# CobaltCrabby/ray_tracer

Measured on AMD Instinct MI355X. Metric: Mrays/s (reference-semantics closest-hit queries) at 1920x1080 Sponza, higher is better.
Workload: dtype f32; 1 GPU; sponza (synthetic-262267-tris), 1920x1080, 8 spp/step, bounceLimit 8, rows interleaved over 1 GPU(s), up to 10 steps in flight per rank (groups of 10+9+9+9); scene=sponza, assets=synthetic-262267-tris, width=1920, height=1080, frames_in_flight=10, pipeline=multi-kernel (k_trace_pw + k_shade per round)

## Files before the change

ray_tracer_amd/csrc/rt_device.hip:

```cpp

#include "rt_kernels.hip.h"
#include "bvh_build.hip.h"

#include <dlfcn.h>
#include <rccl/rccl.h>

#include <algorithm>
#include <chrono>
#include <cmath>
#include <cstdio>
#include <cstdlib>
#include <string>
#include <type_traits>
#include <vector>

namespace {

struct DevBuf {
    void* p = nullptr;
    size_t bytes = 0;
    DevBuf() = default;
    DevBuf(DevBuf&& o) noexcept : p(o.p), bytes(o.bytes) { o.p = nullptr; o.bytes = 0; }
    ~DevBuf() { release(); }
    void release() { if (p) (void)hipFree(p); p = nullptr; bytes = 0; }
};

struct EventPair { hipEvent_t a, b; };
#define RT_MAX_LANES 4
#define RT_FRAMES_MAX_SLOTS (24ull << 20)
struct RowsOf {
    uint32_t width = 0, height = 0, row0 = 0, rowStride = 0, nRows = 0;
    bool whole(uint32_t w, uint32_t h) const { return width == w && height == h && row0 == 0 && rowStride == 1 && nRows == h; }
};

}

struct rt_ctx {
    std::string error;
    int device = 0, numCUs = 256;
    hipStream_t ownStream = nullptr, stream = nullptr;
    DevScene sc{};
    std::vector<DevBuf> sceneBufs;
    DevBuf texelBuf, texInfoBuf, triUVBuf, objTreeBuf, objCostBuf;
    DevBuf matBuf, sphereBuf, sphereMatBuf, objInvBuf, objFwdBuf, objMetaBuf, objBoxBuf, objSkipBuf, maskBoxBuf, emitBuf, emitPreBuf;
    SceneSources host;
    DevBuf objAlphaBuf;
    uint32_t maxLeafDepth = 0;
    std::vector<RootInfo> rootOf;
    bool cull = false;
    ncclComm_t comm = nullptr;
    int commRanks = 0, commRank = 0;
    DevBuf gatherBuf;
    DevBuf stateBuf, queueBuf, fbBuf, counterBuf, scratchBuf;
    DevBuf overflowBuf[RT_MAX_LANES];
    hipStream_t sideStream[RT_MAX_LANES - 1] = {};
    hipEvent_t forkEvent = nullptr, joinEvent[RT_MAX_LANES - 1] = {}, pollEventSide[RT_MAX_LANES - 1] = {};
    uint32_t capacity = 0;
    PathState ps{}; Queues q{};
    uint32_t* hostCounts = nullptr;
    uint32_t fbPixels = 0; bool fbValid = false;
    bool profiling = false;
    std::vector<EventPair> evPool;
    size_t evUsed = 0;
    hipEvent_t profBase = nullptr;
    DevCounters* snap = nullptr;
    hipEvent_t snapEvent = nullptr;
    hipEvent_t pollEvent = nullptr;
    DevBuf probeBuf;
    DevBuf waveTimeBuf;
    DevBuf aovBuf, aovCounterBuf;
    DevBuf shadeStatBuf;
    uint32_t aovPixels = 0; bool aovValid = false;
    RowsOf fbRows, aovRows;
    DevBuf dnWorkBuf, dnHostBuf, dnOutBuf;
// ... 347 lines not shown
    c->meas.snapSeg = seg;
    c->meas.snapPaths = paths;
}
void request_ray_cost(rt_ctx* c) {
    if (c->meas.snapPending) return;
    if (hipMemcpyAsync(c->snap, c->counterBuf.p, sizeof(DevCounters), hipMemcpyDeviceToHost, c->stream) != hipSuccess) return;
    if (hipEventRecord(c->snapEvent, c->stream) != hipSuccess) return;
    c->meas.snapPending = true;
}
void measured_new_scene(rt_ctx* c) {
    if (c->meas.snapPending) { c->meas.snapBox = c->snap->boxTests; c->meas.snapRays = c->snap->raysTraced; c->meas.snapPending = false; }
    c->meas.boxPerRay = -1.0;
}

int harvest_events(rt_ctx* c) {
    for (size_t i = 0; i < c->evUsed; i++) {
        float ms = 0.f;
        RT_HIP(c, hipEventElapsedTime(&ms, c->evPool[i].a, c->evPool[i].b));
        c->rep.traceMs += ms;
        c->rep.traceLaunches++;
        float t0 = 0.f;
        if (c->profBase && hipEventElapsedTime(&t0, c->profBase, c->evPool[i].a) == hipSuccess) c->rep.traceSpans.emplace_back(t0, t0 + ms);
    }
    c->evUsed = 0;
    return 0;
}

int rebuild_emitters(rt_ctx* c) {
    c->sc.emitCount = 0; c->sc.emitSphereMask = 0; c->sc.emitMode = 0;
    const MapLayout maps = layout_maps(c->host, c->sc.texCount);
    int rc = upload_table(c, c->objAlphaBuf, maps.objAlpha, c->sc.objAlpha);
    if (rc) return rc;
    c->sc.mapFlags = maps.mapFlags;
    if (!c->tune.lightQueries) return 0;
    const EmitterLayout e = layout_emitters(c->host, c->rootOf, c->sc.texCount);
    if (!e.mode) return 0;
    if (!e.tris.empty()) {
        if ((rc = upload_table(c, c->emitBuf, e.tris, c->sc.emitTris))) return rc;
    } else {
        if ((rc = dev_alloc(c, c->emitBuf, 256))) return rc;
        c->sc.emitTris = (const uint2*)c->emitBuf.p;
    }
    if ((rc = dev_alloc(c, c->emitPreBuf, std::max<size_t>(e.tris.size(), 1) * 4 * sizeof(float4)))) return rc;
    if (!e.tris.empty()) {
        hipLaunchKernelGGL(k_emit_precompute, dim3(((uint32_t)e.tris.size() + 63u) / 64u), dim3(64), 0, c->stream, c->sc.triPos, c->sc.emitTris, (uint32_t)e.tris.size(), (float4*)c->emitPreBuf.p);
        RT_HIP(c, hipGetLastError());
        RT_HIP(c, hipStreamSynchronize(c->stream));
    }
    c->sc.emitPre = (const float4*)c->emitPreBuf.p;
    c->sc.emitCount = (uint32_t)e.tris.size();
    c->sc.emitSphereMask = e.sphereMask;
    c->sc.emitMode = 1;
    return 0;
}

int set_materials(rt_ctx* c, const RayMaterial* m, uint32_t n) {
    int rc = upload_table(c, c->matBuf, layout_materials(m, n), c->sc.mats);
    if (rc) return rc;
    c->sc.materialCount = n;
    c->host.mats.assign(m, m + n);
    return rebuild_emitters(c);
}

int set_spheres(rt_ctx* c, const Sphere* s, uint32_t n) {
    const SphereLayout l = layout_spheres(s, n);
    int rc = upload_table(c, c->sphereBuf, l.spheres, c->sc.spheres);
    if (rc) return rc;
    if ((rc = upload_table(c, c->sphereMatBuf, l.mat, c->sc.sphereMat))) return rc;
    c->sc.sphereCount = n;
    c->sc.sphereTestMask = l.testMask;
    c->host.sphereMat.assign(l.mat.begin(), l.mat.begin() + n);
    return rebuild_emitters(c);
}

int set_objects(rt_ctx* c, const ObjectLayout& l, const RenderObject* o, uint32_t n) {
    if (l.treeLevels && getenv("RT_DEBUG_OBJTREE")) dump_object_tree(l, n);
    int rc;
    if ((rc = upload_table(c, c->objInvBuf, l.inv, c->sc.objInv))) return rc;
    if ((rc = upload_table(c, c->objFwdBuf, l.fwd, c->sc.objFwd))) return rc;
    if ((rc = upload_table(c, c->objMetaBuf, l.meta, c->sc.objMeta))) return rc;
    if ((rc = upload_table(c, c->objBoxBuf, l.box, c->sc.objBox))) return rc;
    if ((rc = upload_table(c, c->maskBoxBuf, l.maskBox, c->sc.maskBox))) return rc;
    if ((rc = upload_table(c, c->objSkipBuf, l.skipCost, c->sc.objSkipCost))) return rc;
    if ((rc = upload_table(c, c->objTreeBuf, l.tree, c->sc.objTree))) return rc;
    if ((rc = upload_table(c, c->objCostBuf, l.cost, c->sc.objCost))) return rc;
    for (int k = 0; k <= RT_OBJTREE_LEVELS; k++) c->sc.objTreeOff[k] = l.treeOff[k];
    c->sc.objTreeLevels = l.treeLevels;
    c->sc.reachCount = l.reachCount;
    c->sc.maskBase = l.maskBase;
    c->sc.cullOriginLimit = l.cullOriginLimit;
    c->cull = l.cull;
    c->sc.objectCount = n;
    c->host.objMat.resize(n); c->host.objRoot.resize(n); c->host.objSampler.resize(n);
    for (uint32_t i = 0; i < n; i++) { c->host.objMat[i] = o[i].materialIndex; c->host.objRoot[i] = o[i].bvhIndex; c->host.objSampler[i] = o[i].samplerIndex; }
    return rebuild_emitters(c);
}

}

extern "C" {

int rt_device_count(int* out) {
    int n = 0;
    hipError_t e = hipGetDeviceCount(&n);
    if (out) *out = (e == hipSuccess) ? n : 0;
    return e == hipSuccess ? 0 : -1;
}

int rt_create(int device, rt_ctx** out) {
    if (!out) return -1;
    *out = nullptr;
    int n = 0;
    if (hipGetDeviceCount(&n) != hipSuccess || n <= 0) return -2;
    if (device < 0 || device >= n) return -3;
    if (hipSetDevice(device) != hipSuccess) return -4;
    rt_ctx* c = new rt_ctx();
    c->device = device;
    if (hipStreamCreateWithFlags(&c->ownStream, hipStreamNonBlocking) != hipSuccess) { c->ownStream = nullptr; rt_destroy(c); return -5; }
    c->stream = c->ownStream;
    {
        hipDeviceProp_t prop;
        if (hipGetDeviceProperties(&prop, device) == hipSuccess && prop.multiProcessorCount > 0) c->numCUs = prop.multiProcessorCount;
    }
    if (hipHostMalloc((void**)&c->hostCounts, 64, hipHostMallocDefault) != hipSuccess) { c->hostCounts = nullptr; rt_destroy(c); return -6; }
    if (hipHostMalloc((void**)&c->snap, sizeof(DevCounters), hipHostMallocDefault) != hipSuccess) { c->snap = nullptr; rt_destroy(c); return -6; }
    if (hipEventCreateWithFlags(&c->snapEvent, hipEventDisableTiming) != hipSuccess) { c->snapEvent = nullptr; rt_destroy(c); return -6; }
    if (hipEventCreateWithFlags(&c->pollEvent, hipEventDisableTiming) != hipSuccess) { c->pollEvent = nullptr; rt_destroy(c); return -6; }
// ... 185 lines not shown
    for (int l = 0; l < nLanes; l++) {
        const uint32_t u = units / (uint32_t)nLanes + ((uint32_t)l < units % (uint32_t)nLanes ? 1u : 0u);
        const uint32_t end = std::min(nSlots, at + u * unit);
        lane[l] = Lane{d, l ? c->pollEventSide[l - 1] : c->pollEvent, at, end - at, end - at, 0, false, end == at};
        lane[l].d.stream = l ? c->sideStream[l - 1] : c->stream; lane[l].d.counts = c->q.counts + 16 * l; lane[l].d.part = l;
        at = end;
    }
    const int gridPct = part_grid_pct(c->tune, nLanes, lane[0].n);
    for (int l = 0; l < nLanes; l++) lane[l].d.gridPct = gridPct;
}

int render_rounds(rt_ctx* c, const FrameParams& fp, Lane* lane, int nLanes) {
    DevCounters* dc = (DevCounters*)c->counterBuf.p;
    int rc = 0;
    if (nLanes > 1) {
        RT_HIP(c, hipEventRecord(c->forkEvent, c->stream));
        for (int l = 1; l < nLanes; l++) RT_HIP(c, hipStreamWaitEvent(lane[l].d.stream, c->forkEvent, 0));
    }
    const uint64_t maxRounds = (uint64_t)fp.samples * ((uint64_t)fp.bounceLimit + 1);
    for (uint64_t it = 0; it < maxRounds; it++) {
        bool any = false;
        for (int l = 0; l < nLanes; l++) {
            Lane& L = lane[l];
            if (L.done) continue;
            any = true;
            const hipStream_t stream = L.d.stream; uint32_t* const counts = L.d.counts;
            const int cur = L.cur, nxt = cur ^ 1;
            uint32_t* const active[2] = {c->q.active[0] + L.begin, c->q.active[1] + L.begin};
            uint32_t* const rays[2] = {c->q.rays[0] + 3 * (size_t)L.begin, c->q.rays[1] + 3 * (size_t)L.begin};
            hipLaunchKernelGGL(k_zero_counts, dim3(1), dim3(64), 0, stream, counts + nxt, counts + 2 + nxt, counts + 4, counts + 5 + nxt, counts + 7 + nxt);
            TraceArgs ta{rays[cur], counts + 2 + cur, nullptr, nullptr, dc, counts + 5 + cur, counts + 7 + cur, L.n};
            const uint64_t ubRays = std::min<uint64_t>((uint64_t)L.ubActive * 3, (uint64_t)L.n * 3);
            if ((rc = launch_trace(c, L.d, (uint32_t)ubRays, ta))) break;
            ShadeArgs sa{active[cur], counts + cur, active[nxt], rays[nxt], counts + nxt, counts + 2 + nxt, (ShadeStatStripe*)c->shadeStatBuf.p, counts + 5 + nxt, counts + 7 + nxt, L.n};
            if (L.d.sc.mapFlags & (RT_MAP_METALNESS | RT_MAP_BUMP)) hipLaunchKernelGGL(k_shade_maps, dim3((L.ubActive + RT_BLOCK - 1) / RT_BLOCK), dim3(RT_BLOCK), 0, stream, L.d.sc, c->ps, sa, fp);
            else hipLaunchKernelGGL(k_shade, dim3((L.ubActive + RT_BLOCK - 1) / RT_BLOCK), dim3(RT_BLOCK), 0, stream, L.d.sc, c->ps, sa, fp);
            L.cur = nxt;
            if (L.pollPending && hipEventQuery(L.poll) == hipSuccess) {
                L.pollPending = false;
                L.ubActive = std::min(L.ubActive, c->hostCounts[8 + l]);
                if (L.ubActive == 0) { L.done = true; continue; }
            }
            if (!L.pollPending && (it & 7u) == 7u) {
                if (hipMemcpyAsync(c->hostCounts + 8 + l, counts + L.cur, 4, hipMemcpyDeviceToHost, stream) == hipSuccess &&
                    hipEventRecord(L.poll, stream) == hipSuccess)
                    L.pollPending = true;
            }
        }
        if (!any || rc) break;
    }
    for (int l = 1; l < nLanes; l++) {
        RT_HIP(c, hipEventRecord(c->joinEvent[l - 1], lane[l].d.stream));
        RT_HIP(c, hipStreamWaitEvent(c->stream, c->joinEvent[l - 1], 0));
    }
    hipLaunchKernelGGL(k_fold_shade_stats, dim3(1), dim3(RT_STAT_STRIPES), 0, c->stream, (ShadeStatStripe*)c->shadeStatBuf.p, dc);
    return rc;
}

int render_parts(rt_ctx* c, const FrameParams& fp, const Dispatch& d, uint32_t nSlots, float4* fb) {
    const int nLanes = ensure_part_streams(c, choose_parts(c->tune, d, c->cull, c->meas.boxPerRay, fp.samples, nSlots));
    c->rep.lastParts = nLanes;
    Lane lane[RT_MAX_LANES];
    slice_parts(c, d, nSlots, fp.nFrames, nLanes, lane);
    for (int l = 0; l < nLanes; l++) {
        const Lane& L = lane[l];
        if (!L.n) continue;
        hipLaunchKernelGGL(k_raygen, dim3((L.n + RT_BLOCK - 1) / RT_BLOCK), dim3(RT_BLOCK), 0, c->stream, d.sc, c->ps,
// ... 862 lines not shown
```

ray_tracer_amd/csrc/rt_kernels.hip.h:

```cpp
#pragma once

#include <hip/hip_runtime.h>
#include <stdint.h>

#include "rt_amd.h"
#include "rt_det_math.h"
#include "rt_probe.h"
#include "scene_layout.h"

#define RT_WAVE 64
#ifndef RT_QUEUE_ORDER
#define RT_QUEUE_ORDER 0
#endif
#ifndef RT_TE_REG
#define RT_TE_REG 1
#endif
#ifndef RT_OBJTREE
#define RT_OBJTREE 1
#endif
#ifndef RT_SHADE_IDENT
#define RT_SHADE_IDENT 1
#endif
#ifndef RT_FUSED_MAPS_BLOCKS
#define RT_FUSED_MAPS_BLOCKS 4
#endif
#define RT_BLOCK 256
#define RT_HIT_NONE 0xffffffffu
#define RT_HIT_SPHERE 0x80000000u

struct DevScene {
    const float4* nodes;
    const float4* nodesPk;
    const uint32_t* leafFirst;
    const float4* triPos;
    const float4* triNrm;
// ... 57 lines not shown
struct Queues {
    uint32_t* active[2];
    uint32_t* rays[2];
    uint32_t* counts;
};

struct FrameParams {
    float camRot[16];
    float camPos[3];
    float planeWidth, planeHeight;
    float bottomLeft[3];
    uint32_t width, height, row0, rowStride, nRows, nPixels;
    uint32_t tiled;
    uint32_t startingSeed;
    uint32_t samples, bounceLimit;
    uint32_t progressive, frameCount;
    uint32_t camReuse;
    uint32_t nFrames;
    int32_t debug;
    uint32_t boxCap, triCap;
    EnvironmentData env;
};

struct DevCounters {
    unsigned long long boxTests, triTests, raysTraced, raysHit, raysReference, paths, segments, emitterTests;
    unsigned long long skippedBoxTests;
};

#define RT_STAT_STRIPES 256u
struct ShadeStatStripe {
    unsigned long long raysReference, paths, segments, emitterTests;
    unsigned long long pad[12];
};

#define RT_AS_CONSTANT __attribute__((address_space(4)))
#define RT_AS_GLOBAL __attribute__((address_space(1)))
#define RT_AS_LDS __attribute__((address_space(3)))
typedef float rt_f4v __attribute__((ext_vector_type(4)));
typedef float rt_f2v __attribute__((ext_vector_type(2)));
template <typename T> __device__ __forceinline__ const T* rt_uniform(const T* p) { return (const T*)(const RT_AS_CONSTANT T*)(unsigned long long)p; }
template <typename T> __device__ __forceinline__ const T* rt_global(const T* p) { return (const T*)(const RT_AS_GLOBAL T*)(unsigned long long)p; }

__device__ __forceinline__ rt_vec3 f4xyz(float4 v) { return rt_v3(v.x, v.y, v.z); }
__device__ __forceinline__ float4 mk4(rt_vec3 v, float w) { return make_float4(v.x, v.y, v.z, w); }
__device__ __forceinline__ float4 mk4u(rt_vec3 v, uint32_t w) { return make_float4(v.x, v.y, v.z, __uint_as_float(w)); }

__device__ __forceinline__ rt_vec3 xform_dir_rows(float4 r0, float4 r1, float4 r2, rt_vec3 v) {
    return rt_v3((r0.x * v.x + r0.y * v.y) + r0.z * v.z, (r1.x * v.x + r1.y * v.y) + r1.z * v.z,
                 (r2.x * v.x + r2.y * v.y) + r2.z * v.z);
}
__device__ __forceinline__ rt_vec3 xform_point_rows(float4 r0, float4 r1, float4 r2, rt_vec3 v) {
    return rt_v3(((r0.x * v.x + r0.y * v.y) + r0.z * v.z) + r0.w, ((r1.x * v.x + r1.y * v.y) + r1.z * v.z) + r1.w,
                 ((r2.x * v.x + r2.y * v.y) + r2.z * v.z) + r2.w);
}

__device__ __forceinline__ uint32_t lane_id() { return __lane_id(); }
__device__ __forceinline__ uint32_t lanes_below(unsigned long long m) {
    return __builtin_amdgcn_mbcnt_hi((uint32_t)(m >> 32), __builtin_amdgcn_mbcnt_lo((uint32_t)m, 0u));
}
__device__ __forceinline__ unsigned long long wave_sum_u64(unsigned long long v) {
#pragma unroll
    for (int o = 32; o > 0; o >>= 1) v += __shfl_xor(v, o, RT_WAVE);
    return v;
}
__device__ __forceinline__ uint32_t wave_sum_u32(uint32_t v) {
#pragma unroll
// ... 748 lines not shown
    trace_pw_block<STACK, OVF, PIX, STATS, CULL, HOT, BLOCKS == 5, false>(sc, ps, ta);
}
template <bool PIX>
__global__ __launch_bounds__(RT_BLOCK, 4) void k_trace_pw_alpha(DevScene sc, PathState ps, TracePwArgs ta) {
    trace_pw_block<24, true, PIX, false, true, 0, true, true>(sc, ps, ta);
}

struct FullHit {
    rt_vec3 hitPoint, normal;
    uint32_t materialIndex;
    bool frontFace;
    float u, v;
};

__device__ __forceinline__ rt_vec3 albedo_texel(const DevScene& sc, uint32_t slot, uint32_t tri, uint32_t obj, rt_vec3 ro, rt_vec3 rd) {
    float bu, bv, bw;
    {
        const float4 i0 = rt_global(sc.objInv)[3 * obj], i1 = rt_global(sc.objInv)[3 * obj + 1], i2 = rt_global(sc.objInv)[3 * obj + 2];
        const float4 p0 = rt_global(sc.triPos)[3 * (size_t)tri], p1 = rt_global(sc.triPos)[3 * (size_t)tri + 1], p2 = rt_global(sc.triPos)[3 * (size_t)tri + 2];
        const TriHit h = tri_intersect(xform_point_rows(i0, i1, i2, ro), xform_dir_rows(i0, i1, i2, rd), f4xyz(p0), f4xyz(p1), f4xyz(p2), __float_as_uint(p0.w) != 0u);
        bu = h.u; bv = h.v; bw = h.w;
    }
    const float4 a = rt_global(sc.triUV)[2 * (size_t)tri], b = rt_global(sc.triUV)[2 * (size_t)tri + 1];
    float u = (bw * a.x + bu * a.z) + bv * b.x, v = (bw * a.y + bu * a.w) + bv * b.y;
    const bool e01 = a.x == a.z && a.y == a.w, e12 = a.z == b.x && a.w == b.y, e20 = b.x == a.x && b.y == a.y;
    if (e01 || e12 || e20) { u = 0.5f; v = 0.5f; }
    const uint4 ti = rt_global(sc.texInfo)[slot];
    const bool clampEdge = ((rt_global(sc.objMeta)[obj].w >> RT_OBJ_SAMPLER_SHIFT) & RT_OBJ_SAMPLER_MASK) == 1u;
    const uint32_t x = rt_tex_index(u, ti.y, clampEdge), y = rt_tex_index(1.f - v, ti.z, clampEdge);
    const uint32_t t = rt_global(sc.texels)[(size_t)ti.x + (size_t)y * ti.y + x];
    return rt_v3(rt_srgb8_to_linear(t & 0xffu), rt_srgb8_to_linear((t >> 8) & 0xffu), rt_srgb8_to_linear((t >> 16) & 0xffu));
}

template <bool MAPS = false>
__device__ __forceinline__ FullHit reconstruct_hit(const DevScene& sc, rt_vec3 ro, rt_vec3 rd, uint32_t obj, uint32_t tri) {
    FullHit f;
    f.u = 0.f; f.v = 0.f;
    if (obj & RT_HIT_SPHERE) {
        uint32_t i = obj & ~RT_HIT_SPHERE;
        float4 s = rt_global(sc.spheres)[i];
        SphereHit h = sphere_intersect(s, ro, rd);
        f.hitPoint = rt_add(ro, rt_scale(rd, h.dst));
        f.normal = rt_scale(rt_normalize(rt_sub(f.hitPoint, f4xyz(s))), h.frontFace ? 1.f : -1.f);
        f.materialIndex = rt_global(sc.sphereMat)[i];
        f.frontFace = h.frontFace;
        return f;
    }
    const uint4 meta = rt_global(sc.objMeta)[obj];
    const bool ident = RT_SHADE_IDENT && (meta.w & RT_OBJ_FWD_IDENTITY) && ray_is_plain(ro, rd);
    rt_vec3 trd = rd, tro = ro;
    if (!ident) {
        const float4* inv = rt_global(sc.objInv) + 3 * obj;
        const float4 i0 = inv[0], i1 = inv[1], i2 = inv[2];
        trd = xform_dir_rows(i0, i1, i2, rd);
        tro = xform_point_rows(i0, i1, i2, ro);
    }
    const float4* tp = rt_global(sc.triPos) + 3 * (size_t)tri;
    float4 a = tp[0], b = tp[1], c = tp[2];
    TriHit h = tri_intersect(tro, trd, f4xyz(a), f4xyz(b), f4xyz(c), __float_as_uint(a.w) != 0u);
    const float4* tn = rt_global(sc.triNrm) + 3 * (size_t)tri;
    rt_vec3 n0 = f4xyz(tn[0]), n1 = f4xyz(tn[1]), n2 = f4xyz(tn[2]);
    rt_vec3 ni = rt_add(rt_add(rt_scale(n0, h.w), rt_scale(n1, h.u)), rt_scale(n2, h.v));
    if (MAPS) {
        const HitUV q = hit_uv(sc, tri, h.u, h.v, h.w);
        f.u = q.u; f.v = q.v;
        const uint32_t bumpSlot = __float_as_uint(rt_global(sc.mats)[3 * meta.z + 2].w);
// ... 24 lines not shown
__device__ __forceinline__ uint32_t hit_material(const DevScene& sc, uint32_t obj) {
    return (obj & RT_HIT_SPHERE) ? rt_global(sc.sphereMat)[obj & ~RT_HIT_SPHERE] : rt_global(sc.objMeta)[obj].z;
}

__device__ __forceinline__ float schlick(float cosine, float ri) {
    float r0 = (1.f - ri) / (1.f + ri);
    r0 = r0 * r0;
    return r0 + (1.f - r0) * rt_pow(1.f - cosine, 5.f);
}

__device__ __forceinline__ rt_vec3 environment_light(const EnvironmentData& env, rt_vec3 d) {
    if (!(env.lightDir[3] == 1.f)) return rt_v3(0.f, 0.f, 0.f);
    float skyT = rt_pow(rt_smoothstep(0.f, 0.4f, -d.y), 0.35f);
    rt_vec3 sky = rt_v3(rt_mix(env.horizonColor[0], env.zenithColor[0], skyT), rt_mix(env.horizonColor[1], env.zenithColor[1], skyT),
                        rt_mix(env.horizonColor[2], env.zenithColor[2], skyT));
    rt_vec3 negL = rt_v3(-env.lightDir[0], -env.lightDir[1], -env.lightDir[2]);
    float sun = rt_pow(rt_max(0.f, rt_dot(d, negL)), env.horizonColor[3]) * env.zenithColor[3];
    float g2s = rt_smoothstep(-0.01f, 0.f, -d.y);
    float sunMask = g2s >= 1.f ? 1.f : 0.f;
    float add = sun * sunMask;
    return rt_v3(rt_mix(env.groundColor[0], sky.x, g2s) + add, rt_mix(env.groundColor[1], sky.y, g2s) + add,
                 rt_mix(env.groundColor[2], sky.z, g2s) + add);
}

__device__ __forceinline__ float light_cos(rt_vec3 dir) { return rt_dot(rt_v3(0.f, -1.f, 0.f), dir); }
__device__ __forceinline__ float light_sample_pdf(const DevScene& sc, float t, uint32_t obj, float cosTheta) {
    if (obj == RT_HIT_NONE) return 0.f;
    uint32_t m = hit_material(sc, obj);
    if (rt_global(sc.mats)[3 * m + 1].w == 0.f) return 0.f;
    float sq = t * t;
    return sq / (cosTheta * 0.4444444f);
}

__device__ __forceinline__ rt_vec3 primary_dir(const FrameParams& fp, uint32_t gx, uint32_t gy) {
    float u = (float)gx / (float)fp.width;
    float v = (float)gy / (float)fp.height;
    rt_vec3 point = rt_add(rt_v3(fp.bottomLeft[0], fp.bottomLeft[1], fp.bottomLeft[2]),
                           rt_v3(fp.planeWidth * u, fp.planeHeight * v, 0.f));
    rt_vec3 dir = rt_normalize(point);
    return rt_xform_point(fp.camRot, dir);
}

__device__ __forceinline__ uint32_t slot_frame(const FrameParams& fp, uint32_t slot) { return (slot >> 6) % fp.nFrames; }
__device__ __forceinline__ uint32_t slot_in_tile(const FrameParams& fp, uint32_t slot) { return ((slot >> 6) / fp.nFrames << 6) | (slot & 63u); }
__device__ __forceinline__ uint32_t frame_slot(const FrameParams& fp, uint32_t frame, uint32_t tileSlot) {
    return ((tileSlot >> 6) * fp.nFrames + frame) * 64u + (tileSlot & 63u);
}

__device__ __forceinline__ void slot_to_pixel(const FrameParams& fp, uint32_t slot, uint32_t& gx, uint32_t& gy, uint32_t& k) {
    if (fp.nFrames > 1u) slot = slot_in_tile(fp, slot);
    const uint32_t tiledSlots = fp.tiled ? (fp.nRows & ~7u) * fp.width : 0u;
    if (slot < tiledSlots) {
        const uint32_t tile = slot >> 6, in = slot & 63u;
        const uint32_t tilesPerRow = fp.width >> 3;
        const uint32_t tyb = tile / tilesPerRow, txb = tile - tyb * tilesPerRow;
        gx = (txb << 3) + (in & 7u);
        k = (tyb << 3) + (in >> 3);
    } else {
        k = slot / fp.width;
        gx = slot - k * fp.width;
    }
    gy = fp.row0 + k * fp.rowStride;
}

__device__ __forceinline__ void init_path(const DevScene& sc, const PathState& ps, const FrameParams& fp, uint32_t slot) {
    uint32_t gx, gy;
// ... 13 lines not shown
    ps.total()[slot] = make_float4(0.f, 0.f, 0.f, __uint_as_float(0u));
    ps.accum()[slot] = make_float4(0.f, 0.f, 0.f, 0.f);
    ps.statBox()[slot] = 0;
    ps.statTri()[slot] = 0;
}

#define RT_QUEUE_HOLE 0xffffffffu
__global__ __launch_bounds__(RT_BLOCK) void k_raygen(DevScene sc, PathState ps, uint32_t* activeOut, uint32_t* raysOut, FrameParams fp,
                                                     uint32_t slotBegin, uint32_t slotEnd) {
    const uint32_t pos = blockIdx.x * RT_BLOCK + threadIdx.x;
    const uint32_t slot = slotBegin + pos;
    if (slot >= slotEnd) return;
    if (fp.nFrames > 1u && slot_in_tile(fp, slot) >= fp.nPixels) {
        activeOut[pos] = RT_QUEUE_HOLE;
        raysOut[pos] = RT_QUEUE_HOLE;
        return;
    }
    init_path(sc, ps, fp, slot);
    activeOut[pos] = slot;
    raysOut[pos] = slot << 2;
}

struct ShadeArgs {
    const uint32_t* inActive;
    const uint32_t* inCount;
    uint32_t* outActive;
    uint32_t* outRays;
    uint32_t* outActiveCount;
    uint32_t* outRayCount;
    ShadeStatStripe* stats;
    uint32_t* outAuxCount;
    uint32_t* outAuxCount2;
    uint32_t auxOffset;
};

template <bool MAPS = false, bool QUEUED = false>
__device__ __forceinline__ void shade_path(const DevScene& sc, const PathState& ps, const FrameParams& fp, uint32_t slot, bool& alive,
                                           uint32_t& auxMask, uint32_t& refRays, uint32_t& nPaths, uint32_t& emitTests, bool withMask = true) {
    bool wantAux = false;
    auxMask = 0;
    rt_vec3 auxOrigin = rt_v3(0, 0, 0), auxL = auxOrigin, auxC = auxOrigin;
    rt_vec3 auxAlbedo = auxOrigin;
    float auxNdotL = 0.f, auxCosPdfL = 0.f, auxCosPdfC = 0.f;
    float auxCosL = 0.f, auxCosC = 0.f;
    const float4 sO = ps.rayO()[slot], sD = ps.rayD()[slot], sA = ps.att()[slot], sT = ps.total()[slot];
    const float4 hM = (QUEUED && fp.camReuse && (__float_as_uint(sA.w) & 0x0fffffffu) == 0u && __float_as_uint(sT.w) != 0u) ? ps.camHit()[slot]
                                                                                                                        : ps.hit(RAY_MAIN)[slot];
    rt_vec3 ro = f4xyz(sO), rd = f4xyz(sD);
    rt_vec3 att = f4xyz(sA), total = f4xyz(sT);
    float misW = sO.w;
    uint32_t state = __float_as_uint(sD.w);
    uint32_t jraw = __float_as_uint(sA.w);
    uint32_t samplesDone = __float_as_uint(sT.w);
    uint32_t j = jraw & 0x0fffffffu;
    const bool pending = (jraw >> 31) != 0u;
    rt_vec3 direct = (jraw & 0x40000000u) ? rt_v3(-1.f, -1.f, -1.f) : rt_v3(0.f, 0.f, 0.f);
    bool specular = false;

    const uint32_t obj = __float_as_uint(hM.y);
    const uint32_t hitTriIdx = __float_as_uint(hM.z);
    refRays = 1;
    if (fp.camReuse && j == 0u && samplesDone == 0u) ps.camHit()[slot] = hM;

    bool done = false;
    bool zeroed = false;

    if (obj != RT_HIT_NONE) {
        if (pending) {
            float4 hL = make_float4(RT_MISS_DST, __uint_as_float(RT_HIT_NONE), 0.f, 0.f), hC = hL;
            if (!(jraw & 0x20000000u)) hL = ps.hit(RAY_NEE)[slot];
            if (!(jraw & 0x10000000u)) hC = ps.hit(RAY_PROBE)[slot];
            const float4 pM = ps.pendMis()[slot];
            float tL = hL.x, tC = hC.x;
            uint32_t oL = __float_as_uint(hL.y), oC = __float_as_uint(hC.y);
            uint32_t lm = (oL == RT_HIT_NONE) ? 0u : hit_material(sc, oL);
            float4 lmE = rt_global(sc.mats)[3 * lm + 1];
            float realLightPDF = light_sample_pdf(sc, tL, oL, pM.x);
            float cosinePDF = pM.z;
            float misWeight1 = realLightPDF * realLightPDF / (realLightPDF * realLightPDF + cosinePDF * cosinePDF);
            if (rt_isnan(misWeight1)) misWeight1 = 0.f;
            float lightPDF = light_sample_pdf(sc, tC, oC, pM.y);
            float realCosinePDF = pM.w;
            float misWeight2 = realCosinePDF * realCosinePDF / (lightPDF * lightPDF + realCosinePDF * realCosinePDF);
            if (rt_isnan(misWeight2)) misWeight2 = 0.f;
            const float4 pA = ps.pendAlbedo()[slot];
            rt_vec3 albedo = f4xyz(pA);
            rt_vec3 dl = rt_scale(rt_v3(lmE.x, lmE.y, lmE.z), lmE.w);
            float k = (realLightPDF == 0.f) ? 0.f : misWeight1 / realLightPDF;
            rt_vec3 f = rt_scale(rt_scale(rt_scale(albedo, RT_INV_PI), pA.w), k);
            direct = rt_mul(dl, f);
            misW = misWeight2;
        }

        FullHit hit = reconstruct_hit<MAPS>(sc, ro, rd, obj, hitTriIdx);
        const float4* mp = rt_global(sc.mats) + 3 * hit.materialIndex;
        float4 mA = mp[0], mE = mp[1], mI = mp[2];
        if (MAPS) {
            const uint32_t metalSlot = __float_as_uint(mI.z);
            if (metalSlot < sc.texCount && !(obj & RT_HIT_SPHERE))
                mA.w = rt_srgb8_to_linear(map_red8(sc, metalSlot, ((rt_global(sc.objMeta)[obj].w >> RT_OBJ_SAMPLER_SHIFT) & RT_OBJ_SAMPLER_MASK) == 1u, hit.u, hit.v, false, false));
        }

        rt_vec3 emission = rt_scale(rt_v3(mE.x, mE.y, mE.z), mE.w);
        emission = rt_v3(emission.x / misW, emission.y / misW, emission.z / misW);
        rt_vec3 finalLight = direct.x == -1.f ? emission : direct;
        total = rt_add(total, rt_mul(finalLight, att));
        if (j == 0) total = rt_add(total, emission);
        if (rt_isnan(total.x) || rt_isnan(total.y) || rt_isnan(total.z) || total.x < 0.f || total.y < 0.f || total.z < 0.f) {
            done = true;
            zeroed = true;
        } else {
            rt_vec3 sampledDir, radiance;
            float originSign = 1.f;
            bool diffuse = false;
            if (mA.w != 0.f) {
                sampledDir = rt_reflect(rd, hit.normal);
                radiance = rt_v3(1.f, 1.f, 1.f);
                specular = true;
// ... 122 lines not shown
                if (auxMask & 2u) ps.auxDC()[slot] = mk4(auxC, 0.f);
                ps.pendAlbedo()[slot] = mk4(auxAlbedo, auxNdotL);
                ps.pendMis()[slot] = make_float4(auxCosL, auxCosC, auxCosPdfL, auxCosPdfC);
            }
        }
        const uint32_t answered = wantAux ? (((auxMask & 1u) ? 0u : 0x20000000u) | ((auxMask & 2u) ? 0u : 0x10000000u)) : 0u;
        ps.rayO()[slot] = mk4(ro, misW);
        ps.rayD()[slot] = mk4u(rd, state);
        ps.att()[slot] = mk4u(att, j | (wantAux ? 0x80000000u : 0u) | (specular ? 0x40000000u : 0u) | answered);
        const float4 nT = mk4u(total, samplesDone);
        if (!QUEUED || __float_as_uint(nT.x) != __float_as_uint(sT.x) || __float_as_uint(nT.y) != __float_as_uint(sT.y) ||
            __float_as_uint(nT.z) != __float_as_uint(sT.z) || __float_as_uint(nT.w) != __float_as_uint(sT.w))
            ps.total()[slot] = nT;
    }
}

template <bool MAPS>
__device__ __forceinline__ void shade_block(const DevScene& sc, const PathState& ps, const ShadeArgs& sa, const FrameParams& fp) {
    __shared__ uint32_t s_cnt[RT_BLOCK / RT_WAVE][8];
    __shared__ uint32_t s_base[4];
    const uint32_t n = *sa.inCount;
    if (blockIdx.x * RT_BLOCK >= n) return;
    const uint32_t gid = blockIdx.x * RT_BLOCK + threadIdx.x;
    const bool live = gid < n;

    bool alive = false;
    uint32_t auxMask = 0;
    uint32_t slot = 0;
    uint32_t refRays = 0, nPaths = 0, emitTests = 0;
    bool path = live;
    if (live) {
        slot = sa.inActive[gid];
        path = slot != 0xffffffffu;
        if (path) shade_path<MAPS, true>(sc, ps, fp, slot, alive, auxMask, refRays, nPaths, emitTests);
    }

    const unsigned long long mAlive = __ballot(alive), mM = __ballot(alive && !(auxMask & 4u));
    const unsigned long long mL = __ballot(alive && (auxMask & 1u)), mC = __ballot(alive && (auxMask & 2u));
    const uint32_t nAlive = __popcll(mAlive), nM = __popcll(mM), nL = __popcll(mL), nC = __popcll(mC);
    const uint32_t wRef = wave_sum_u32(refRays), wPaths = wave_sum_u32(nPaths), wSeg = wave_sum_u32(path ? 1u : 0u), wEmit = wave_sum_u32(emitTests);
    const uint32_t wv = threadIdx.x / RT_WAVE;
    if (lane_id() == 0) {
        s_cnt[wv][0] = nAlive; s_cnt[wv][1] = nM; s_cnt[wv][2] = wRef; s_cnt[wv][3] = wPaths; s_cnt[wv][4] = wSeg; s_cnt[wv][5] = wEmit; s_cnt[wv][6] = nL; s_cnt[wv][7] = nC;
    }
    __syncthreads();
    if (threadIdx.x == 0) {
        uint32_t tA = 0, tR = 0, tRef = 0, tP = 0, tS = 0, tE = 0, tX = 0, tY = 0;
        for (int w = 0; w < RT_BLOCK / RT_WAVE; w++) { tA += s_cnt[w][0]; tR += s_cnt[w][1]; tRef += s_cnt[w][2]; tP += s_cnt[w][3]; tS += s_cnt[w][4]; tE += s_cnt[w][5]; tX += s_cnt[w][6]; tY += s_cnt[w][7]; }
        s_base[0] = tA ? atomicAdd(sa.outActiveCount, tA) : 0u;
        s_base[1] = tR ? atomicAdd(sa.outRayCount, tR) : 0u;
        s_base[2] = tX ? atomicAdd(RT_QUEUE_ORDER ? sa.outAuxCount2 : sa.outAuxCount, tX) : 0u;
        s_base[3] = tY ? atomicAdd(RT_QUEUE_ORDER ? sa.outAuxCount : sa.outAuxCount2, tY) : 0u;
        ShadeStatStripe* const st = sa.stats + (blockIdx.x & (RT_STAT_STRIPES - 1u));
        atomicAdd(&st->raysReference, (unsigned long long)tRef);
        if (tP) atomicAdd(&st->paths, (unsigned long long)tP);
        atomicAdd(&st->segments, (unsigned long long)tS);
        if (tE) atomicAdd(&st->emitterTests, (unsigned long long)tE);
    }
    __syncthreads();
    if (alive) {
        uint32_t baseA = s_base[0], baseR = s_base[1];
        uint32_t baseX = (RT_QUEUE_ORDER ? 2u : 1u) * sa.auxOffset + s_base[2], baseY = (RT_QUEUE_ORDER ? 1u : 2u) * sa.auxOffset + s_base[3];
        for (uint32_t w = 0; w < wv; w++) { baseA += s_cnt[w][0]; baseR += s_cnt[w][1]; baseX += s_cnt[w][6]; baseY += s_cnt[w][7]; }
        sa.outActive[baseA + lanes_below(mAlive)] = slot;
        if (!(auxMask & 4u)) sa.outRays[baseR + lanes_below(mM)] = (slot << 2) | ((auxMask & 8u) ? RAY_MAIN_BLANK : (uint32_t)RAY_MAIN);
        if (auxMask & 1u) sa.outRays[baseX + lanes_below(mL)] = (slot << 2) | RAY_NEE;
        if (auxMask & 2u) sa.outRays[baseY + lanes_below(mC)] = (slot << 2) | RAY_PROBE;
    }
}

__global__ __launch_bounds__(RT_BLOCK) void k_shade(DevScene sc, PathState ps, ShadeArgs sa, FrameParams fp) { shade_block<false>(sc, ps, sa, fp); }
__global__ __launch_bounds__(RT_BLOCK) void k_shade_maps(DevScene sc, PathState ps, ShadeArgs sa, FrameParams fp) { shade_block<true>(sc, ps, sa, fp); }

__device__ __forceinline__ rt_vec3 blend_frame(const FrameParams& fp, uint32_t frameCount, float4 oldc, float4 accum) {
    rt_vec3 out = f4xyz(accum);
    float fs = (float)fp.samples;
    out = rt_v3(out.x / fs, out.y / fs, out.z / fs);
    float weight = 1.f / ((float)frameCount + 1.f);
    rt_vec3 blended = rt_add(rt_scale(rt_v3(oldc.x, oldc.y, oldc.z), 1.f - weight), rt_scale(out, weight));
    rt_vec3 fin = fp.progressive ? blended : out;
    if (rt_isnan(fin.x) || rt_isnan(fin.y) || rt_isnan(fin.z) || rt_isinf(fin.x) || rt_isinf(fin.y) || rt_isinf(fin.z))
        fin = rt_v3(1.f, 0.f, 1.f);
    return fin;
}

__device__ __forceinline__ void resolve_pixel(const PathState& ps, const FrameParams& fp, float4* rgba, uint32_t slot) {
    uint32_t gx, gy, krow;
    slot_to_pixel(fp, slot, gx, gy, krow);
    const size_t px = (size_t)krow * fp.width + gx;
    rt_vec3 fin = blend_frame(fp, fp.frameCount, rgba[px], ps.accum()[slot]);
// ... 334 lines not shown
```

ray_tracer_amd/csrc/scene_layout.cpp:

```cpp

#include "scene_layout.h"

#include <algorithm>
#include <cmath>
#include <cstdio>
#include <cstring>
#include <utility>

#include "rt_det_math.h"

namespace {

float4 with_w(float x, float y, float z, uint32_t w) {
    float4 v = make_float4(x, y, z, 0.f);
    memcpy(&v.w, &w, 4);
    return v;
}

void rows_of(const float* m, float4* out) {
    for (int r = 0; r < 3; r++) out[r] = make_float4(m[0 + r], m[4 + r], m[8 + r], m[12 + r]);
}

bool rows_are_identity(const float4* rows) {
    static const float ident[12] = {1, 0, 0, 0, 0, 1, 0, 0, 0, 0, 1, 0};
// ... 294 lines not shown
}

TextureLayout layout_textures(const RtTexture* tex, uint32_t n) {
    TextureLayout l;
    if (n > (uint32_t)RT_MAX_TEXTURES) { l.error = "more than RT_MAX_TEXTURES textures"; return l; }
    l.info.assign(std::max(n, 1u), make_uint4(0u, 1u, 1u, 0u));
    size_t total = 0;
    for (uint32_t i = 0; i < n; i++) {
        if (!tex[i].rgba8 || tex[i].width == 0 || tex[i].height == 0) { l.error = "texture " + std::to_string(i) + " is empty"; return l; }
        if ((uint64_t)tex[i].width * tex[i].height > (1ull << 28) || total + (size_t)tex[i].width * tex[i].height > 0xffffffffull) { l.error = "textures too large"; return l; }
        l.info[i] = make_uint4((uint32_t)total, tex[i].width, tex[i].height, 0u);
        total += (size_t)tex[i].width * tex[i].height;
    }
    l.texels.assign(std::max<size_t>(total, 1), 0u);
    for (uint32_t i = 0; i < n; i++) memcpy(&l.texels[l.info[i].x], tex[i].rgba8, (size_t)tex[i].width * tex[i].height * 4);
    return l;
}

MapLayout layout_maps(const SceneSources& src, uint32_t texCount) {
    MapLayout l;
    const uint32_t n = (uint32_t)src.objMat.size();
    auto bound = [&](int32_t index) { return index >= 0 && (uint32_t)index < texCount; };
    l.objAlpha.assign(std::max(n, 1u), RT_OBJALPHA_NONE);
    for (uint32_t i = 0; i < n; i++) {
        if (src.objMat[i] >= src.mats.size()) continue;
        const RayMaterial& m = src.mats[src.objMat[i]];
        if (bound(m.metalnessIndex)) l.mapFlags |= RT_MAP_METALNESS;
        if (bound(m.bumpIndex)) l.mapFlags |= RT_MAP_BUMP;
        if (bound(m.alphaIndex)) { l.mapFlags |= RT_MAP_ALPHA; l.objAlpha[i] = (uint32_t)m.alphaIndex | (src.objSampler[i] == 1u ? RT_OBJALPHA_CLAMP : 0u); }
    }
    return l;
}

EmitterLayout layout_emitters(const SceneSources& src, const std::vector<RootInfo>& rootOf, uint32_t texCount) {
    const EmitterLayout none;
    EmitterLayout l;
    if (src.mats.empty()) return none;
    auto emissive = [&](uint32_t m) { return m < src.mats.size() && !(src.mats[m].emissionStrength == 0.f); };
    for (const RayMaterial& m : src.mats)
        for (int k = 0; k < 3; k++)
            if (!std::isfinite(m.emissionColor[k] * m.emissionStrength)) return none;
    for (size_t i = 0; i < src.sphereMat.size() && i < 32; i++)
        if (emissive(src.sphereMat[i])) l.sphereMask |= 1u << i;
    for (size_t i = 32; i < src.sphereMat.size(); i++)
        if (emissive(src.sphereMat[i])) return none;
    for (size_t i = 0; i < src.objMat.size(); i++) {
        if (!emissive(src.objMat[i])) continue;
        { const int32_t ai = src.mats[src.objMat[i]].alphaIndex; if (ai >= 0 && (uint32_t)ai < texCount) return none; }
        const RootInfo& r = rootOf[src.objRoot[i]];
        if (r.triTotal == 0xffffffffu || l.tris.size() + r.triTotal > (size_t)RT_EMIT_MAX_TRIS) return none;
        for (uint32_t t = 0; t < r.triTotal; t++) l.tris.push_back(make_uint2((uint32_t)i, r.triFirst + t));
    }
    l.mode = 1;
    return l;
}
```

ray_tracer_amd/csrc/scene_layout.h:

```cpp
#pragma once

#include <hip/hip_vector_types.h>
#include <stdint.h>

#include <string>
#include <vector>

#include "rt_amd.h"

#define RT_LEAF_BIT 0x80000000u
#define RT_LEAF_CNT_SHIFT 28
#define RT_LEAF_IDX_MASK 0x0fffffffu
#define RT_HOT_PAIRS 192u
#define RT_OBJTREE_LEVELS 8

#define RT_OBJ_IDENTITY 1u
#define RT_OBJ_BOX 2u
#define RT_OBJ_MASKABLE 4u
#define RT_OBJ_FWD_IDENTITY 8u
#define RT_OBJ_SAMPLER_SHIFT 16
#define RT_OBJ_SAMPLER_MASK 0xffffu
#define RT_OBJALPHA_NONE 0xffffffffu
#define RT_OBJALPHA_SLOT_MASK 0xffu
#define RT_OBJALPHA_CLAMP 0x100u
// ... 24 lines not shown
    bool cull = false;
};
ObjectLayout layout_objects(const RenderObject* o, uint32_t n, const std::vector<RootInfo>& rootOf, uint32_t materialCount,
                            int objTreeMin, int maskIdentity);
void dump_object_tree(const ObjectLayout& l, uint32_t n);

struct SceneLayout {
    std::string error;
    MeshLayout meshes;
    ObjectLayout objects;
};
SceneLayout layout_scene(const RtSceneArrays& s, int objTreeMin, int maskIdentity);

std::vector<float4> layout_materials(const RayMaterial* m, uint32_t n);

struct SphereLayout {
    std::vector<float4> spheres;
    std::vector<uint32_t> mat;
    uint32_t testMask = 0;
};
SphereLayout layout_spheres(const Sphere* s, uint32_t n);

struct TextureLayout {
    std::string error;
    std::vector<uint4> info;
    std::vector<uint32_t> texels;
};
TextureLayout layout_textures(const RtTexture* tex, uint32_t n);

struct SceneSources {
    std::vector<RayMaterial> mats;
    std::vector<uint32_t> sphereMat, objMat, objRoot, objSampler;
};
struct MapLayout {
    std::vector<uint32_t> objAlpha;
    uint32_t mapFlags = 0;
};
MapLayout layout_maps(const SceneSources& src, uint32_t texCount);

struct EmitterLayout {
    uint32_t mode = 0, sphereMask = 0;
    std::vector<uint2> tris;
};
EmitterLayout layout_emitters(const SceneSources& src, const std::vector<RootInfo>& rootOf, uint32_t texCount);
```

Before: 4718 Mrays/s.

## Index emission by hit id and prefetch pending NEE data in queued shade

Adds a host-built per-hit emission table, appended to the material buffer, indexed directly by object or sphere hit id. This lets the queued shade path skip the hit-to-material indirection before reading emission. It also issues the pending NEE, probe, MIS and albedo loads early through branchless address selection, and spreads the per-block counter and statistics atomics across eight threads instead of one. The cost is an extra table upload on every scene change and possible extra loads of a dummy array for non-pending slots.

```diff
diff --git a/ray_tracer_amd/csrc/rt_device.hip b/ray_tracer_amd/csrc/rt_device.hip
--- a/ray_tracer_amd/csrc/rt_device.hip
+++ b/ray_tracer_amd/csrc/rt_device.hip
@@ -40,6 +40,7 @@
     int device = 0, numCUs = 256;
     hipStream_t ownStream = nullptr, stream = nullptr;
     DevScene sc{};
+    HitEmission hitEmit{};
     std::vector<DevBuf> sceneBufs;
     DevBuf texelBuf, texInfoBuf, triUVBuf, objTreeBuf, objCostBuf;
     DevBuf matBuf, sphereBuf, sphereMatBuf, objInvBuf, objFwdBuf, objMetaBuf, objBoxBuf, objSkipBuf, maskBoxBuf, emitBuf, emitPreBuf;
@@ -453,6 +454,12 @@
     int rc = upload_table(c, c->objAlphaBuf, maps.objAlpha, c->sc.objAlpha);
     if (rc) return rc;
     c->sc.mapFlags = maps.mapFlags;
+    const HitEmissionLayout hm = layout_hit_emission(c->host);
+    std::vector<float4> mats = layout_materials(c->host.mats.data(), (uint32_t)c->host.mats.size());
+    const size_t hitBase = mats.size();
+    mats.insert(mats.end(), hm.emit.begin(), hm.emit.end());
+    if ((rc = upload_table(c, c->matBuf, mats, c->sc.mats))) return rc;
+    c->hitEmit = HitEmission{c->sc.mats + hitBase, hm.sphereBase, hm.none};
     if (!c->tune.lightQueries) return 0;
     const EmitterLayout e = layout_emitters(c->host, c->rootOf, c->sc.texCount);
     if (!e.mode) return 0;
@@ -476,11 +483,13 @@
 }
 
 int set_materials(rt_ctx* c, const RayMaterial* m, uint32_t n) {
-    int rc = upload_table(c, c->matBuf, layout_materials(m, n), c->sc.mats);
-    if (rc) return rc;
+    std::vector<RayMaterial> before = c->host.mats;
+    const uint32_t countBefore = c->sc.materialCount;
     c->sc.materialCount = n;
-    c->host.mats.assign(m, m + n);
-    return rebuild_emitters(c);
+    sources_set_materials(c->host, m, n);
+    const int rc = rebuild_emitters(c);
+    if (rc) { c->host.mats.swap(before); c->sc.materialCount = countBefore; }
+    return rc;
 }
 
 int set_spheres(rt_ctx* c, const Sphere* s, uint32_t n) {
@@ -490,7 +499,7 @@
     if ((rc = upload_table(c, c->sphereMatBuf, l.mat, c->sc.sphereMat))) return rc;
     c->sc.sphereCount = n;
     c->sc.sphereTestMask = l.testMask;
-    c->host.sphereMat.assign(l.mat.begin(), l.mat.begin() + n);
+    sources_set_spheres(c->host, s, n);
     return rebuild_emitters(c);
 }
 
@@ -512,8 +521,7 @@
     c->sc.cullOriginLimit = l.cullOriginLimit;
     c->cull = l.cull;
     c->sc.objectCount = n;
-    c->host.objMat.resize(n); c->host.objRoot.resize(n); c->host.objSampler.resize(n);
-    for (uint32_t i = 0; i < n; i++) { c->host.objMat[i] = o[i].materialIndex; c->host.objRoot[i] = o[i].bvhIndex; c->host.objSampler[i] = o[i].samplerIndex; }
+    sources_set_objects(c->host, o, n);
     return rebuild_emitters(c);
 }
 
@@ -765,7 +773,7 @@
             TraceArgs ta{rays[cur], counts + 2 + cur, nullptr, nullptr, dc, counts + 5 + cur, counts + 7 + cur, L.n};
             const uint64_t ubRays = std::min<uint64_t>((uint64_t)L.ubActive * 3, (uint64_t)L.n * 3);
             if ((rc = launch_trace(c, L.d, (uint32_t)ubRays, ta))) break;
-            ShadeArgs sa{active[cur], counts + cur, active[nxt], rays[nxt], counts + nxt, counts + 2 + nxt, (ShadeStatStripe*)c->shadeStatBuf.p, counts + 5 + nxt, counts + 7 + nxt, L.n};
+            ShadeArgs sa{active[cur], counts + cur, active[nxt], rays[nxt], counts + nxt, counts + 2 + nxt, (ShadeStatStripe*)c->shadeStatBuf.p, counts + 5 + nxt, counts + 7 + nxt, L.n, c->hitEmit};
             if (L.d.sc.mapFlags & (RT_MAP_METALNESS | RT_MAP_BUMP)) hipLaunchKernelGGL(k_shade_maps, dim3((L.ubActive + RT_BLOCK - 1) / RT_BLOCK), dim3(RT_BLOCK), 0, stream, L.d.sc, c->ps, sa, fp);
             else hipLaunchKernelGGL(k_shade, dim3((L.ubActive + RT_BLOCK - 1) / RT_BLOCK), dim3(RT_BLOCK), 0, stream, L.d.sc, c->ps, sa, fp);
             L.cur = nxt;
diff --git a/ray_tracer_amd/csrc/rt_kernels.hip.h b/ray_tracer_amd/csrc/rt_kernels.hip.h
--- a/ray_tracer_amd/csrc/rt_kernels.hip.h
+++ b/ray_tracer_amd/csrc/rt_kernels.hip.h
@@ -1,6 +1,7 @@
 #pragma once
 
 #include <hip/hip_runtime.h>
+#include <stddef.h>
 #include <stdint.h>
 
 #include "rt_amd.h"
@@ -124,6 +125,8 @@
     unsigned long long raysReference, paths, segments, emitterTests;
     unsigned long long pad[12];
 };
+static_assert(offsetof(ShadeStatStripe, paths) == 8 && offsetof(ShadeStatStripe, segments) == 16 && offsetof(ShadeStatStripe, emitterTests) == 24,
+              "shade_block indexes the four statistics from raysReference");
 
 #define RT_AS_CONSTANT __attribute__((address_space(4)))
 #define RT_AS_GLOBAL __attribute__((address_space(1)))
@@ -938,6 +941,15 @@
     return rt_v3(rt_srgb8_to_linear(t & 0xffu), rt_srgb8_to_linear((t >> 8) & 0xffu), rt_srgb8_to_linear((t >> 16) & 0xffu));
 }
 
+struct HitEmission {
+    const float4* emit;
+    uint32_t sphereBase, none;
+};
+__device__ __forceinline__ uint32_t hit_table_index(const HitEmission& he, uint32_t obj) {
+    return obj == RT_HIT_NONE ? he.none : (obj & RT_HIT_SPHERE) ? he.sphereBase + (obj & ~RT_HIT_SPHERE) : obj;
+}
+__device__ __forceinline__ float4 hit_emission(const HitEmission& he, uint32_t obj) { return rt_global(he.emit)[hit_table_index(he, obj)]; }
+
 template <bool MAPS = false>
 __device__ __forceinline__ FullHit reconstruct_hit(const DevScene& sc, rt_vec3 ro, rt_vec3 rd, uint32_t obj, uint32_t tri) {
     FullHit f;
@@ -1028,6 +1040,13 @@
     return sq / (cosTheta * 0.4444444f);
 }
 
+__device__ __forceinline__ float light_sample_pdf_of(float t, uint32_t obj, float emissionStrength, float cosTheta) {
+    if (obj == RT_HIT_NONE) return 0.f;
+    if (emissionStrength == 0.f) return 0.f;
+    float sq = t * t;
+    return sq / (cosTheta * 0.4444444f);
+}
+
 __device__ __forceinline__ rt_vec3 primary_dir(const FrameParams& fp, uint32_t gx, uint32_t gy) {
     float u = (float)gx / (float)fp.width;
     float v = (float)gy / (float)fp.height;
@@ -1107,11 +1126,13 @@
     uint32_t* outAuxCount;
     uint32_t* outAuxCount2;
     uint32_t auxOffset;
+    HitEmission hitEmit;
 };
 
 template <bool MAPS = false, bool QUEUED = false>
 __device__ __forceinline__ void shade_path(const DevScene& sc, const PathState& ps, const FrameParams& fp, uint32_t slot, bool& alive,
-                                           uint32_t& auxMask, uint32_t& refRays, uint32_t& nPaths, uint32_t& emitTests, bool withMask = true) {
+                                           uint32_t& auxMask, uint32_t& refRays, uint32_t& nPaths, uint32_t& emitTests, bool withMask = true,
+                                           const HitEmission& he = HitEmission{nullptr, 0u, 0u}) {
     bool wantAux = false;
     auxMask = 0;
     rt_vec3 auxOrigin = rt_v3(0, 0, 0), auxL = auxOrigin, auxC = auxOrigin;
@@ -1121,6 +1142,18 @@
     const float4 sO = ps.rayO()[slot], sD = ps.rayD()[slot], sA = ps.att()[slot], sT = ps.total()[slot];
     const float4 hM = (QUEUED && fp.camReuse && (__float_as_uint(sA.w) & 0x0fffffffu) == 0u && __float_as_uint(sT.w) != 0u) ? ps.camHit()[slot]
                                                                                                                         : ps.hit(RAY_MAIN)[slot];
+    float4 bL, bC, bM, bA;
+    if (QUEUED) {
+        const uint32_t w = __float_as_uint(sA.w);
+        const bool pend = (w >> 31) != 0u;
+        uint32_t ownArray = 8u;
+        asm volatile("" : "+s"(ownArray));
+        const float4* const own = ps.arr(ownArray) + slot;
+        bL = *((pend && !(w & 0x20000000u)) ? ps.hit(RAY_NEE) + slot : own);
+        bC = *((pend && !(w & 0x10000000u)) ? ps.hit(RAY_PROBE) + slot : own);
+        bM = *(pend ? ps.pendMis() + slot : own);
+        bA = *(pend ? ps.pendAlbedo() + slot : own);
+    }
     rt_vec3 ro = f4xyz(sO), rd = f4xyz(sD);
     rt_vec3 att = f4xyz(sA), total = f4xyz(sT);
     float misW = sO.w;
@@ -1143,22 +1176,24 @@
     if (obj != RT_HIT_NONE) {
         if (pending) {
             float4 hL = make_float4(RT_MISS_DST, __uint_as_float(RT_HIT_NONE), 0.f, 0.f), hC = hL;
-            if (!(jraw & 0x20000000u)) hL = ps.hit(RAY_NEE)[slot];
-            if (!(jraw & 0x10000000u)) hC = ps.hit(RAY_PROBE)[slot];
-            const float4 pM = ps.pendMis()[slot];
+            if (!(jraw & 0x20000000u)) hL = QUEUED ? bL : ps.hit(RAY_NEE)[slot];
+            if (!(jraw & 0x10000000u)) hC = QUEUED ? bC : ps.hit(RAY_PROBE)[slot];
+            const float4 pM = QUEUED ? bM : ps.pendMis()[slot];
             float tL = hL.x, tC = hC.x;
             uint32_t oL = __float_as_uint(hL.y), oC = __float_as_uint(hC.y);
-            uint32_t lm = (oL == RT_HIT_NONE) ? 0u : hit_material(sc, oL);
-            float4 lmE = rt_global(sc.mats)[3 * lm + 1];
-            float realLightPDF = light_sample_pdf(sc, tL, oL, pM.x);
+            constexpr bool BY_HIT = QUEUED;
+            uint32_t lm = (BY_HIT || oL == RT_HIT_NONE) ? 0u : hit_material(sc, oL);
+            float4 lmE = BY_HIT ? hit_emission(he, oL) : rt_global(sc.mats)[3 * lm + 1];
+            const float cmS = BY_HIT ? hit_emission(he, oC).w : 0.f;
+            float realLightPDF = BY_HIT ? light_sample_pdf_of(tL, oL, lmE.w, pM.x) : light_sample_pdf(sc, tL, oL, pM.x);
             float cosinePDF = pM.z;
             float misWeight1 = realLightPDF * realLightPDF / (realLightPDF * realLightPDF + cosinePDF * cosinePDF);
             if (rt_isnan(misWeight1)) misWeight1 = 0.f;
-            float lightPDF = light_sample_pdf(sc, tC, oC, pM.y);
+            float lightPDF = BY_HIT ? light_sample_pdf_of(tC, oC, cmS, pM.y) : light_sample_pdf(sc, tC, oC, pM.y);
             float realCosinePDF = pM.w;
             float misWeight2 = realCosinePDF * realCosinePDF / (lightPDF * lightPDF + realCosinePDF * realCosinePDF);
             if (rt_isnan(misWeight2)) misWeight2 = 0.f;
-            const float4 pA = ps.pendAlbedo()[slot];
+            const float4 pA = QUEUED ? bA : ps.pendAlbedo()[slot];
             rt_vec3 albedo = f4xyz(pA);
             rt_vec3 dl = rt_scale(rt_v3(lmE.x, lmE.y, lmE.z), lmE.w);
             float k = (realLightPDF == 0.f) ? 0.f : misWeight1 / realLightPDF;
@@ -1347,7 +1382,7 @@
     if (live) {
         slot = sa.inActive[gid];
         path = slot != 0xffffffffu;
-        if (path) shade_path<MAPS, true>(sc, ps, fp, slot, alive, auxMask, refRays, nPaths, emitTests);
+        if (path) shade_path<MAPS, true>(sc, ps, fp, slot, alive, auxMask, refRays, nPaths, emitTests, true, sa.hitEmit);
     }
 
     const unsigned long long mAlive = __ballot(alive), mM = __ballot(alive && !(auxMask & 4u));
@@ -1359,18 +1394,23 @@
         s_cnt[wv][0] = nAlive; s_cnt[wv][1] = nM; s_cnt[wv][2] = wRef; s_cnt[wv][3] = wPaths; s_cnt[wv][4] = wSeg; s_cnt[wv][5] = wEmit; s_cnt[wv][6] = nL; s_cnt[wv][7] = nC;
     }
     __syncthreads();
-    if (threadIdx.x == 0) {
-        uint32_t tA = 0, tR = 0, tRef = 0, tP = 0, tS = 0, tE = 0, tX = 0, tY = 0;
-        for (int w = 0; w < RT_BLOCK / RT_WAVE; w++) { tA += s_cnt[w][0]; tR += s_cnt[w][1]; tRef += s_cnt[w][2]; tP += s_cnt[w][3]; tS += s_cnt[w][4]; tE += s_cnt[w][5]; tX += s_cnt[w][6]; tY += s_cnt[w][7]; }
-        s_base[0] = tA ? atomicAdd(sa.outActiveCount, tA) : 0u;
-        s_base[1] = tR ? atomicAdd(sa.outRayCount, tR) : 0u;
-        s_base[2] = tX ? atomicAdd(RT_QUEUE_ORDER ? sa.outAuxCount2 : sa.outAuxCount, tX) : 0u;
-        s_base[3] = tY ? atomicAdd(RT_QUEUE_ORDER ? sa.outAuxCount : sa.outAuxCount2, tY) : 0u;
-        ShadeStatStripe* const st = sa.stats + (blockIdx.x & (RT_STAT_STRIPES - 1u));
-        atomicAdd(&st->raysReference, (unsigned long long)tRef);
-        if (tP) atomicAdd(&st->paths, (unsigned long long)tP);
-        atomicAdd(&st->segments, (unsigned long long)tS);
-        if (tE) atomicAdd(&st->emitterTests, (unsigned long long)tE);
+    if (threadIdx.x < 8u) {
+        const uint32_t k = threadIdx.x;
+        const uint32_t col = k < 2u ? k : (k < 4u ? k + 4u : k - 2u);
+        uint32_t t = 0;
+        for (int w = 0; w < RT_BLOCK / RT_WAVE; w++) t += s_cnt[w][col];
+        if (k < 4u) {
+            uint32_t* const cX = RT_QUEUE_ORDER ? sa.outAuxCount2 : sa.outAuxCount;
+            uint32_t* const cY = RT_QUEUE_ORDER ? sa.outAuxCount : sa.outAuxCount2;
+            uint32_t* const counter = k == 0u ? sa.outActiveCount : k == 1u ? sa.outRayCount : k == 2u ? cX : cY;
+            uint32_t base = 0u;
+            if (t) base = atomicAdd(counter, t);
+            s_base[k] = base;
+        } else if (t) {
+            ShadeStatStripe* const st = sa.stats + (blockIdx.x & (RT_STAT_STRIPES - 1u));
+            unsigned long long* const four = &st->raysReference;
+            atomicAdd(four + (k - 4u), (unsigned long long)t);
+        }
     }
     __syncthreads();
     if (alive) {
diff --git a/ray_tracer_amd/csrc/scene_layout.cpp b/ray_tracer_amd/csrc/scene_layout.cpp
--- a/ray_tracer_amd/csrc/scene_layout.cpp
+++ b/ray_tracer_amd/csrc/scene_layout.cpp
@@ -350,6 +350,32 @@
     return l;
 }
 
+void sources_set_materials(SceneSources& src, const RayMaterial* m, uint32_t n) { src.mats.assign(m, m + n); }
+void sources_set_spheres(SceneSources& src, const Sphere* s, uint32_t n) {
+    src.sphereMat.resize(n);
+    for (uint32_t i = 0; i < n; i++) src.sphereMat[i] = s[i].materialIndex;
+}
+void sources_set_objects(SceneSources& src, const RenderObject* o, uint32_t n) {
+    src.objMat.resize(n); src.objRoot.resize(n); src.objSampler.resize(n);
+    for (uint32_t i = 0; i < n; i++) { src.objMat[i] = o[i].materialIndex; src.objRoot[i] = o[i].bvhIndex; src.objSampler[i] = o[i].samplerIndex; }
+}
+
+HitEmissionLayout layout_hit_emission(const SceneSources& src) {
+    HitEmissionLayout l;
+    const uint32_t nObj = (uint32_t)src.objMat.size(), nSph = (uint32_t)src.sphereMat.size();
+    l.sphereBase = std::max(nObj, 1u);
+    l.none = l.sphereBase + std::max(nSph, 1u);
+    const std::vector<float4> mats = layout_materials(src.mats.data(), (uint32_t)src.mats.size());
+    l.emit.assign((size_t)l.none + 1, make_float4(0.f, 0.f, 0.f, 0.f));
+    auto put = [&](uint32_t entry, uint32_t m) {
+        if (m < src.mats.size()) l.emit[entry] = mats[3 * (size_t)m + 1];
+    };
+    for (uint32_t i = 0; i < nObj; i++) put(i, src.objMat[i]);
+    for (uint32_t i = 0; i < nSph; i++) put(l.sphereBase + i, src.sphereMat[i]);
+    put(l.none, 0u);
+    return l;
+}
+
 EmitterLayout layout_emitters(const SceneSources& src, const std::vector<RootInfo>& rootOf, uint32_t texCount) {
     const EmitterLayout none;
     EmitterLayout l;
diff --git a/ray_tracer_amd/csrc/scene_layout.h b/ray_tracer_amd/csrc/scene_layout.h
--- a/ray_tracer_amd/csrc/scene_layout.h
+++ b/ray_tracer_amd/csrc/scene_layout.h
@@ -80,12 +80,21 @@
     std::vector<RayMaterial> mats;
     std::vector<uint32_t> sphereMat, objMat, objRoot, objSampler;
 };
+void sources_set_materials(SceneSources& src, const RayMaterial* m, uint32_t n);
+void sources_set_spheres(SceneSources& src, const Sphere* s, uint32_t n);
+void sources_set_objects(SceneSources& src, const RenderObject* o, uint32_t n);
 struct MapLayout {
     std::vector<uint32_t> objAlpha;
     uint32_t mapFlags = 0;
 };
 MapLayout layout_maps(const SceneSources& src, uint32_t texCount);
 
+struct HitEmissionLayout {
+    std::vector<float4> emit;
+    uint32_t sphereBase = 1, none = 2;
+};
+HitEmissionLayout layout_hit_emission(const SceneSources& src);
+
 struct EmitterLayout {
     uint32_t mode = 0, sphereMask = 0;
     std::vector<uint2> tris;
```

New measurement: 4776 Mrays/s (median of 6 runs). 1.2% higher.
